# NIRVANALAN/GaussianAnything

Hardware: NVIDIA H100
Metric: 512^2 views/sec @100k Gaussians (surfel raster fwd+bwd) (higher is better)
Workload: dtype f32

## Files before the change

### gaussiananything_b200/csrc/raster_api.cu

```cuda
#include "../../include/ga_b200.h"
#include "raster_common.cuh"

static size_t align_up(size_t x, size_t a) { return (x + a - 1) / a * a; }

static int g_profile = 0;
static cudaEvent_t g_ev[7];
static bool g_ev_init = false;
static inline void prof(int i, cudaStream_t s) { if (g_profile) cudaEventRecord(g_ev[i], s); }

extern "C" int ga_profile_enable(int on)
{
    if (on && !g_ev_init) {
        for (int i = 0; i < 7; i++)
            if (cudaEventCreate(&g_ev[i]) != cudaSuccess) return GA_ERR_BADARG;
        g_ev_init = true;
    }
    g_profile = on ? 1 : 0;
    return 0;
}

extern "C" int ga_profile_read(float *ms, int n)
{
    if (!g_ev_init || !ms || n < 5) return 0;
    if (cudaEventSynchronize(g_ev[6]) != cudaSuccess) return 0;
// ... 33 lines not shown
}

extern "C" int ga_raster_layout_ex(int batch, int P, int views, int H, int W,
                                   int64_t max_instances, int list_k, GaRasterLayout *L)
{
    RasterDims d;
    int rc = make_dims(batch, P, views, H, W, 1.0f, max_instances, &d, list_k);
    if (rc) return rc;
    if (!L) return GA_ERR_BADARG;
    const size_t NVP = (size_t)d.NV * P, NVT = (size_t)d.NV * d.T, HW = (size_t)H * W;
    const size_t mi = (size_t)(max_instances > 0 ? max_instances : 1);
    size_t off = 0;
    L->status = off;     off = align_up(off + 16 * sizeof(int32_t), 256);
    L->rec = off;        off = align_up(off + NVP * GA_REC_F * sizeof(float), 256);
    L->depth = off;      off = align_up(off + NVP * sizeof(float), 256);
    L->rect = off;       off = align_up(off + NVP * sizeof(uint32_t), 256);
    L->tile_count = off; off = align_up(off + NVT * (GA_TILE_REPLICAS + 1) * sizeof(uint32_t), 256);
    L->tile_start = off; off = align_up(off + (NVT + 1) * sizeof(uint32_t), 256);
    L->keys = off;       off = align_up(off + mi * sizeof(uint64_t), 256);
    L->ids = off;        off = align_up(off + mi * sizeof(uint32_t), 256);
    L->final_T = off;    off = align_up(off + (size_t)d.NV * 3 * HW * sizeof(float), 256);
    L->n_contrib = off;  off = align_up(off + (size_t)d.NV * 2 * HW * sizeof(int32_t), 256);
    L->inst_cnt = off;   off = align_up(off + mi * sizeof(uint32_t), 256);
    L->n_list = off;     off = align_up(off + (list_k ? (size_t)d.NV * HW * sizeof(int32_t) : 0), 256);
    L->tile_flag = off;  off = align_up(off + (list_k ? NVT * sizeof(uint32_t) : 0), 256);
    L->lists = off;      off = align_up(off + (size_t)list_k * NVT * 256 * 16, 256);
    L->total_bytes = off;
    return 0;
}

static void carve(const GaRasterLayout &L, const RasterDims &d, void *base, RasterWs *w)
{
    char *p = (char *)base;
    w->status = (int32_t *)(p + L.status);
    w->rec = (float *)(p + L.rec);
    w->depth = (float *)(p + L.depth);
    w->rect = (uint32_t *)(p + L.rect);
    w->tile_count = (uint32_t *)(p + L.tile_count);
    w->big_tiles = w->tile_count + (size_t)d.NV * d.T * GA_TILE_REPLICAS;
    w->tile_start = (uint32_t *)(p + L.tile_start);
    w->keys = (unsigned long long *)(p + L.keys);
    w->ids = (uint32_t *)(p + L.ids);
    w->final_T = (float *)(p + L.final_T);
    w->n_contrib = (int32_t *)(p + L.n_contrib);
    w->inst_cnt = (uint32_t *)(p + L.inst_cnt);
    w->n_list = (int32_t *)(p + L.n_list);
    w->tile_flag = (uint32_t *)(p + L.tile_flag);
    w->lists = (uint4 *)(p + L.lists);
}

extern "C" int ga_raster_forward_ex(const float *gauss13, int batch, int P, int views,
                                    const float *viewmats, const float *projmats, const float *bg,
                                    int H, int W, float scale_modifier,
                                    float *out_color, float *out_allmap, int32_t *out_radii,
                                    void *workspace, size_t workspace_bytes, int64_t max_instances, int list_k,
                                    int32_t *status_host, void *status_event, void *stream)
{
    if ((status_host == nullptr) != (status_event == nullptr)) return GA_ERR_BADARG;
    RasterDims d;
    int rc = make_dims(batch, P, views, H, W, scale_modifier, max_instances, &d, list_k);
    if (rc) return rc;
    if (!gauss13 || !viewmats || !projmats || !bg || !out_color || !out_allmap || !out_radii || !workspace)
        return GA_ERR_BADARG;
    GaRasterLayout L;
    ga_raster_layout_ex(batch, P, views, H, W, max_instances, list_k, &L);
    if (workspace_bytes < L.total_bytes) return GA_ERR_WORKSPACE;
    RasterWs w;
    carve(L, d, workspace, &w);
    cudaStream_t s = (cudaStream_t)stream;
    cudaError_t e;
    if ((e = cudaMemsetAsync(w.status, 0, 16 * sizeof(int32_t), s)) != cudaSuccess) return (int)e;
    if ((e = cudaMemsetAsync(w.tile_count, 0, (size_t)d.NV * d.T * GA_TILE_REPLICAS * sizeof(uint32_t), s)) != cudaSuccess) return (int)e;
    prof(0, s);
    if ((e = ga_launch_preprocess(d, w, gauss13, viewmats, projmats, out_radii, s)) != cudaSuccess) return (int)e;
    prof(1, s);
    if ((e = ga_launch_binning(d, w, s, status_host, (cudaEvent_t)status_event)) != cudaSuccess) return (int)e;
    prof(2, s);
    if (list_k && (e = cudaMemsetAsync(w.tile_flag, 0, (size_t)d.NV * d.T * sizeof(uint32_t), s)) != cudaSuccess) return (int)e;
    if ((e = ga_launch_render_fwd(d, w, bg, out_color, out_allmap, s)) != cudaSuccess) return (int)e;
    prof(3, s);
    return 0;
}

static size_t bwd_acc_bytes(int batch, int P, int views) { return align_up((size_t)batch * views * P * GA_GRAD_F * sizeof(float), 256); }

extern "C" size_t ga_raster_backward_scratch_bytes(int batch, int P, int views)
{
    if (batch <= 0 || P <= 0 || views <= 0) return 0;
    return bwd_acc_bytes(batch, P, views);
}

extern "C" int ga_raster_backward_ex(const float *gauss13, int batch, int P, int views,
                                     const float *viewmats, const float *projmats, const float *bg,
                                     int H, int W, float scale_modifier,
                                     const int32_t *radii,
                                     const float *dL_dcolor, const float *dL_dallmap,
                                     const void *workspace, size_t workspace_bytes, int64_t max_instances, int list_k,
                                     void *scratch, size_t scratch_bytes,
                                     float *grad_gauss13, void *stream)
{
    RasterDims d;
    int rc = make_dims(batch, P, views, H, W, scale_modifier, max_instances, &d, list_k);
    if (rc) return rc;
    if (!gauss13 || !viewmats || !projmats || !bg || !radii || !dL_dcolor || !dL_dallmap ||
        !workspace || !scratch || !grad_gauss13)
        return GA_ERR_BADARG;
    GaRasterLayout L;
    ga_raster_layout_ex(batch, P, views, H, W, max_instances, list_k, &L);
    if (workspace_bytes < L.total_bytes) return GA_ERR_WORKSPACE;
    const size_t need = bwd_acc_bytes(batch, P, views);
    if (scratch_bytes < need) return GA_ERR_WORKSPACE;
    RasterWs w;
    carve(L, d, const_cast<void *>(workspace), &w);
    cudaStream_t s = (cudaStream_t)stream;
    cudaError_t e;
    float *grad_acc = (float *)scratch;
    prof(4, s);
    if ((e = cudaMemsetAsync(grad_acc, 0, need, s)) != cudaSuccess) return (int)e;
    if ((e = ga_launch_render_bwd(d, w, bg, dL_dcolor, dL_dallmap, grad_acc, s)) != cudaSuccess) return (int)e;
    prof(5, s);
    if ((e = ga_launch_preprocess_bwd(d, w, gauss13, viewmats, projmats, radii, grad_acc, grad_gauss13, s)) != cudaSuccess)
        return (int)e;
    prof(6, s);
    return 0;
}

extern "C" const char *ga_b200_version(void) { return "ga_b200 0.2 (sm_90a)"; }
```

### gaussiananything_b200/csrc/raster_common.cuh

```cuda
#pragma once
#include <cuda_runtime.h>
#include <stdint.h>

#define GA_BLOCK_X 16
#define GA_BLOCK_Y 16
#define GA_NEAR_N 0.2f
#define GA_FAR_N 100.0f
#define GA_FILTER_SIZE 0.707106f
#define GA_FILTER_INV_SQUARE 2.0f
#define GA_CUTOFF 3.0f
#define GA_REC_F 24
#define GA_GRAD_F 18


struct RasterDims {
    int batch, P, views, NV;
    int H, W, gx, gy, T;
    float scale_modifier;
    int64_t max_instances;
    int list_k;
    int radius_formula;
    int quat_norm_grad;
};
#ifndef GA_RADIUS_FORMULA
#define GA_RADIUS_FORMULA 0
#endif
#ifndef GA_QUAT_NORM_GRAD
#define GA_QUAT_NORM_GRAD 0
#endif

struct RasterWs {
    int32_t *status;
    float *rec;
    float *depth;
    uint32_t *rect;
    uint32_t *tile_count;
    uint32_t *big_tiles;
    uint32_t *tile_start;
    unsigned long long *keys;
    uint32_t *ids;
    float *final_T;
    int32_t *n_contrib;
    uint4 *lists;
    int32_t *n_list;
    uint32_t *tile_flag;
    uint32_t *inst_cnt;
};

cudaError_t ga_launch_preprocess(const RasterDims &d, const RasterWs &w, const float *gauss13,
                                 const float *viewmats, const float *projmats,
                                 int32_t *out_radii, cudaStream_t s);
#ifndef GA_TILE_REPLICAS
#define GA_TILE_REPLICAS 8
#endif

cudaError_t ga_launch_binning(const RasterDims &d, const RasterWs &w, cudaStream_t s, int32_t *status_host,
                              cudaEvent_t status_event);
cudaError_t ga_launch_render_fwd(const RasterDims &d, const RasterWs &w, const float *bg,
                                 float *out_color, float *out_allmap, cudaStream_t s);
cudaError_t ga_launch_render_bwd(const RasterDims &d, const RasterWs &w, const float *bg,
                                 const float *dL_dcolor, const float *dL_dallmap,
                                 float *grad_acc, cudaStream_t s);
cudaError_t ga_launch_preprocess_bwd(const RasterDims &d, const RasterWs &w, const float *gauss13,
                                     const float *viewmats, const float *projmats,
                                     const int32_t *radii, const float *grad_acc,
                                     float *grad_gauss13, cudaStream_t s);
```

### gaussiananything_b200/csrc/raster_preprocess.cu

```cuda
#include "raster_common.cuh"

__device__ __forceinline__ void quat_to_rotmat(const float *q, float R[3][3])
{
    float n2 = ((q[0] * q[0] + q[1] * q[1]) + q[2] * q[2]) + q[3] * q[3];
    float s = 1.0f / sqrtf(n2);
    float w = q[0] * s, x = q[1] * s, y = q[2] * s, z = q[3] * s;
    R[0][0] = 1.f - 2.f * (y * y + z * z);
    R[1][0] = 2.f * (x * y + w * z);
    R[2][0] = 2.f * (x * z - w * y);
    R[0][1] = 2.f * (x * y - w * z);
    R[1][1] = 1.f - 2.f * (x * x + z * z);
    R[2][1] = 2.f * (y * z + w * x);
    R[0][2] = 2.f * (x * z + w * y);
    R[1][2] = 2.f * (y * z - w * x);
    R[2][2] = 1.f - 2.f * (x * x + y * y);
}

__device__ __forceinline__ void surfel_transmat(const float R[3][3], float sx, float sy, float px, float py, float pz,
                                                const float *pm, int W, int H, float Tu[3], float Tv[3], float Tw[3])
{
    float L0[3] = {R[0][0] * sx, R[1][0] * sx, R[2][0] * sx};
    float L1[3] = {R[0][1] * sy, R[1][1] * sy, R[2][1] * sy};
    const float hw = 0.5f * (float)W, hh = 0.5f * (float)H;
    const float cw = 0.5f * (float)(W - 1), ch = 0.5f * (float)(H - 1);
// ... 96 lines not shown
                            float hx = sqrtf(fmaxf(0.f, qx)) * 1.01f + 0.51f;
                            float hy = sqrtf(fmaxf(0.f, qy)) * 1.01f + 0.51f;
                            bx0 = fminf(bx0, ccx - hx); bx1 = fmaxf(bx1, ccx + hx);
                            by0 = fminf(by0, ccy - hy); by1 = fmaxf(by1, ccy + hy);
                        } else {
                            bx0 = -1e30f; bx1 = 1e30f; by0 = -1e30f; by1 = 1e30f;
                        }
                    }
                    rec[16] = bx0; rec[17] = bx1; rec[18] = by0; rec[19] = by1;
                }
            }
        }
    }
    out_radii[vi] = radius_i;
    ws.depth[vi] = depth_out;
    ws.rect[vi] = rect_packed;
#pragma unroll
    for (int q = 0; q < GA_REC_F / 4; q++)
        rec_out[q] = make_float4(rec[4 * q], rec[4 * q + 1], rec[4 * q + 2], rec[4 * q + 3]);
    if (radius_i > 0) {
        const int x0 = rect_packed & 255, y0 = (rect_packed >> 8) & 255;
        const int x1 = (rect_packed >> 16) & 255, y1 = rect_packed >> 24;
        uint32_t *tc = ws.tile_count + (size_t)view * d.T * GA_TILE_REPLICAS + ((threadIdx.x >> 5) & (GA_TILE_REPLICAS - 1));
        for (int y = y0; y < y1; y++)
            for (int x = x0; x < x1; x++) atomicAdd(&tc[(y * d.gx + x) * GA_TILE_REPLICAS], 1u);
    }
}

__global__ void __launch_bounds__(256, 4)
preprocess_kernel(RasterDims d, RasterWs ws, const float *__restrict__ gauss13,
                  const float *__restrict__ viewmats, const float *__restrict__ projmats,
                  int32_t *__restrict__ out_radii)
{
    __shared__ float s_g[256 * 13];
    __shared__ float s_cam[32];
    __shared__ float4 s_rec[256 * GA_REC_F / 4];
    const int view = blockIdx.y;
    const int b = view / d.views;
    const int i0 = blockIdx.x * 256;
    const int n = min(256, d.P - i0);
    const float *src = gauss13 + ((size_t)b * d.P + i0) * 13;
    for (int t = threadIdx.x; t < n * 13; t += 256) s_g[t] = src[t];
    if (threadIdx.x < 16) s_cam[threadIdx.x] = viewmats[view * 16 + threadIdx.x];
    else if (threadIdx.x < 32) s_cam[threadIdx.x] = projmats[view * 16 + threadIdx.x - 16];
    __syncthreads();
    if ((int)threadIdx.x < n) preprocess_one(d, ws, s_g + threadIdx.x * 13, s_cam, view, i0 + threadIdx.x,
                                             s_rec + threadIdx.x * (GA_REC_F / 4), out_radii);
    __syncthreads();
    float4 *dst = reinterpret_cast<float4 *>(ws.rec + ((size_t)view * d.P + i0) * GA_REC_F);
    for (int t = threadIdx.x; t < n * (GA_REC_F / 4); t += 256) dst[t] = s_rec[t];
}

cudaError_t ga_launch_preprocess(const RasterDims &d, const RasterWs &w, const float *gauss13,
                                 const float *viewmats, const float *projmats,
                                 int32_t *out_radii, cudaStream_t s)
{
    dim3 grid((d.P + 255) / 256, d.NV);
    preprocess_kernel<<<grid, 256, 0, s>>>(d, w, gauss13, viewmats, projmats, out_radii);
    return cudaGetLastError();
}

__global__ void __launch_bounds__(256)
preprocess_bwd_kernel(RasterDims d, RasterWs ws, const float *__restrict__ gauss13,
                      const float *__restrict__ viewmats, const float *__restrict__ projmats,
                      const int32_t *__restrict__ radii, const float *__restrict__ grad_acc,
                      float *__restrict__ grad_gauss13)
{
    const int b = blockIdx.y;
    const int i = blockIdx.x * 256 + threadIdx.x;
    if (i >= d.P) return;
    const float *g = gauss13 + ((size_t)b * d.P + i) * 13;
    float q[4] = {g[6], g[7], g[8], g[9]};
    float R[3][3];
    quat_to_rotmat(q, R);
    const float sx = d.scale_modifier * g[4], sy = d.scale_modifier * g[5];
    const float px = g[0], py = g[1], pz = g[2];
    const float hw = 0.5f * d.W, hh = 0.5f * d.H, cw = 0.5f * (d.W - 1), ch = 0.5f * (d.H - 1);
    float gm[3] = {0, 0, 0}, gs[2] = {0, 0}, dR[3][3] = {{0, 0, 0}, {0, 0, 0}, {0, 0, 0}};
    float gop = 0.f, gcol[3] = {0, 0, 0};
    for (int v = 0; v < d.views; v++) {
        const int view = b * d.views + v;
        const size_t vi = (size_t)view * d.P + i;
        if (!(radii[vi] > 0)) continue;
        const float *ga = grad_acc + vi * GA_GRAD_F;
        const float *vm = viewmats + view * 16, *pm = projmats + view * 16;
        float G[3][3];
#pragma unroll
        for (int c = 0; c < 3; c++)
#pragma unroll
            for (int r = 0; r < 3; r++) G[c][r] = ga[3 * c + r];
        const float gmx = ga[9], gmy = ga[10];
        if (gmx != 0.f || gmy != 0.f) {
            const float t[3] = {9.f, 9.f, -1.f};
            float Tu[3], Tv[3], Tw[3];
            surfel_transmat(R, sx, sy, px, py, pz, pm, d.W, d.H, Tu, Tv, Tw);
            float dd = 0.f;
#pragma unroll
            for (int r = 0; r < 3; r++) dd += t[r] * Tw[r] * Tw[r];
            float f[3], dL_dd = 0.f;
#pragma unroll
            for (int r = 0; r < 3; r++) f[r] = t[r] / dd;
#pragma unroll
            for (int r = 0; r < 3; r++) {
                G[0][r] += gmx * f[r] * Tw[r];
                G[1][r] += gmy * f[r] * Tw[r];
                G[2][r] += gmx * f[r] * Tu[r] + gmy * f[r] * Tv[r];
                dL_dd += (gmx * Tu[r] * Tw[r] + gmy * Tv[r] * Tw[r]) * f[r];
            }
            dL_dd *= (-1.0f / dd);
#pragma unroll
            for (int r = 0; r < 3; r++) G[2][r] += dL_dd * t[r] * Tw[r] * 2.0f;
        }
        float dM[3][3];
#pragma unroll
        for (int k = 0; k < 3; k++) {
            float an0 = pm[4 * k + 0] * hw + pm[4 * k + 3] * cw;
            float an1 = pm[4 * k + 1] * hh + pm[4 * k + 3] * ch;
            float an2 = pm[4 * k + 3];
#pragma unroll
            for (int r = 0; r < 3; r++) dM[r][k] = an0 * G[0][r] + an1 * G[1][r] + an2 * G[2][r];
        }
        float vx = ((vm[0] * px + vm[4] * py) + vm[8] * pz) + vm[12];
        float vy = ((vm[1] * px + vm[5] * py) + vm[9] * pz) + vm[13];
        float vz = ((vm[2] * px + vm[6] * py) + vm[10] * pz) + vm[14];
        float nx = (vm[0] * R[0][2] + vm[4] * R[1][2]) + vm[8] * R[2][2];
        float ny = (vm[1] * R[0][2] + vm[5] * R[1][2]) + vm[9] * R[2][2];
        float nz = (vm[2] * R[0][2] + vm[6] * R[1][2]) + vm[10] * R[2][2];
        float cosv = -((vx * nx + vy * ny) + vz * nz);
        const float mult = cosv > 0.f ? 1.f : -1.f;
        const float gn0 = ga[11], gn1 = ga[12], gn2 = ga[13];
        float dtn[3];
        dtn[0] = mult * (vm[0] * gn0 + vm[1] * gn1 + vm[2] * gn2);
        dtn[1] = mult * (vm[4] * gn0 + vm[5] * gn1 + vm[6] * gn2);
        dtn[2] = mult * (vm[8] * gn0 + vm[9] * gn1 + vm[10] * gn2);
#pragma unroll
        for (int k = 0; k < 3; k++) {
            dR[k][0] += dM[0][k] * sx;
            dR[k][1] += dM[1][k] * sy;
            dR[k][2] += dtn[k];
            gs[0] += dM[0][k] * R[k][0];
            gs[1] += dM[1][k] * R[k][1];
            gm[k] += dM[2][k];
        }
        gop += ga[14];
        gcol[0] += ga[15]; gcol[1] += ga[16]; gcol[2] += ga[17];
    }
    float n2 = q[0] * q[0] + q[1] * q[1] + q[2] * q[2] + q[3] * q[3];
    float s = rsqrtf(n2);
    float w = q[0] * s, x = q[1] * s, y = q[2] * s, z = q[3] * s;
    float gw = 2 * (z * (dR[1][0] - dR[0][1]) + y * (dR[0][2] - dR[2][0]) + x * (dR[2][1] - dR[1][2]));
    float gxq = 2 * (-2 * x * (dR[1][1] + dR[2][2]) + y * (dR[1][0] + dR[0][1]) + z * (dR[2][0] + dR[0][2]) + w * (dR[2][1] - dR[1][2]));
    float gyq = 2 * (x * (dR[1][0] + dR[0][1]) - 2 * y * (dR[0][0] + dR[2][2]) + z * (dR[2][1] + dR[1][2]) + w * (dR[0][2] - dR[2][0]));
    float gzq = 2 * (x * (dR[2][0] + dR[0][2]) + y * (dR[2][1] + dR[1][2]) - 2 * z * (dR[0][0] + dR[1][1]) + w * (dR[1][0] - dR[0][1]));
    if (d.quat_norm_grad) {
        const float dot = w * gw + x * gxq + y * gyq + z * gzq;
        gw = (gw - w * dot) * s; gxq = (gxq - x * dot) * s; gyq = (gyq - y * dot) * s; gzq = (gzq - z * dot) * s;
    }
    float *o = grad_gauss13 + ((size_t)b * d.P + i) * 13;
    o[0] = gm[0]; o[1] = gm[1]; o[2] = gm[2];
    o[3] = gop;
    o[4] = d.scale_modifier * gs[0]; o[5] = d.scale_modifier * gs[1];
    o[6] = gw; o[7] = gxq; o[8] = gyq; o[9] = gzq;
    o[10] = gcol[0]; o[11] = gcol[1]; o[12] = gcol[2];
}

cudaError_t ga_launch_preprocess_bwd(const RasterDims &d, const RasterWs &w, const float *gauss13,
                                     const float *viewmats, const float *projmats,
// ... 9 lines not shown
```

### gaussiananything_b200/csrc/raster_render.cu

```cuda
#include "raster_common.cuh"
#include "device_once.cuh"

#define CHUNK 256

__device__ __forceinline__ float fast_rcp(float x)
{
    float r;
    asm("rcp.approx.ftz.f32 %0, %1;" : "=f"(r) : "f"(x));
    return r;
}
__device__ __forceinline__ float fast_ex2(float x)
{
    float r;
    asm("ex2.approx.ftz.f32 %0, %1;" : "=f"(r) : "f"(x));
    return r;
}
#define GA_M_C0 (GA_FAR_N / (GA_FAR_N - GA_NEAR_N))
#define GA_M_C1 (GA_FAR_N * GA_NEAR_N / (GA_FAR_N - GA_NEAR_N))
#define GA_NEG_HALF_LOG2E (-0.72134752044448170368f)

struct PixelGeom {
    float s0, s1, p2, rho3d, rho2d, dx, dy, depth, G, alpha;
    bool use3d;
};
// ... 98 lines not shown
            const TileBox q = clip_box(bb, ox, oy, min(ox + 15, d.W - 1), min(oy + 15, d.H - 1));
            npairs = q.w * q.h;
            sm.box[threadIdx.x] = npairs ? (uint32_t)(q.x0 | q.y0 << 4 | q.w << 8 | (65536 / q.w + 1) << 13) : 0u;
        }
        int incl = npairs;
#pragma unroll
        for (int o = 1; o < 32; o <<= 1) {
            const int y = __shfl_up_sync(0xffffffffu, incl, o);
            if (lane >= o) incl += y;
        }
        if (lane == 31) sm.wsum[warp] = incl;
        __syncthreads();
#pragma unroll
        for (int k = 0; k < 8; k++) incl += k < warp ? sm.wsum[k] : 0;
        sm.base[threadIdx.x] = incl - npairs;
        if (threadIdx.x == CHUNK - 1) sm.base[CHUNK] = incl;

        int t0 = 0, base = 0;
        while (t0 < cnt) {
#pragma unroll
            for (int k = 0; k < CHUNK / 32; k++) sm.mask[k][threadIdx.x] = 0u;
            const int t1 = t0 + __syncthreads_count((int)threadIdx.x >= t0 && (int)threadIdx.x < cnt &&
                                                    incl - base <= FWD_PAIRS);
            const int wpairs = sm.base[t1] - base;
            for (int q = threadIdx.x; q < wpairs; q += 256) {
                const int Q = base + q;
                int jj = t0;
#pragma unroll
                for (int step = CHUNK / 2; step > 0; step >>= 1)
                    if (jj + step < t1 && sm.base[jj + step] <= Q) jj += step;
                const uint32_t bx = sm.box[jj];
                const int k = Q - sm.base[jj], w = (bx >> 8) & 31;
                const int ry = (k * (int)(bx >> 13)) >> 16;
                const int lx = (int)(bx & 15) + k - ry * w, ly = (int)((bx >> 4) & 15) + ry;
                const float dxf = (float)lx, dyf = (float)ly;
                const float4 f0 = sm.rec[0][jj], f1 = sm.rec[1][jj], f2 = sm.rec[2][jj], f3 = sm.rec[3][jj];
                const float p0 = f0.x + dxf * f0.w + dyf * f1.z;
                const float p1 = f0.y + dxf * f1.x + dyf * f1.w;
                const float p2 = f0.z + dxf * f1.y + dyf * f2.x;
                const float ip = fast_rcp(p2);
                const float s0 = p0 * ip, s1 = p1 * ip;
                const float rho3d = s0 * s0 + s1 * s1;
                const float ddx = f3.x - dxf, ddy = f3.y - dyf;
                const float rho2d = GA_FILTER_INV_SQUARE * __fmaf_rn(ddx, ddx, __fmul_rn(ddy, ddy));
                const float rho = fminf(rho3d, rho2d);
                const float depth = (rho3d <= rho2d) ? (s0 * f2.y + s1 * f2.z) + f2.w : f2.w;
                const float alpha = fminf(0.99f, f3.z * fast_ex2(rho * GA_NEG_HALF_LOG2E));
                if (p2 != 0.0f && depth >= GA_NEAR_N && alpha >= 1.0f / 255.0f) {
                    sm.pair[q] = make_float2(alpha, depth);
                    atomicOr(&sm.mask[jj >> 5][ly * 16 + lx], 1u << (jj & 31));
                }
            }
            __syncthreads();
            if (!done) {
                int wi = t0 >> 5;
                const int wlast = (t1 - 1) >> 5;
                uint32_t m = sm.mask[wi][pix_local];
                while (true) {
                    while (m == 0u && wi < wlast) m = sm.mask[++wi][pix_local];
                    if (m == 0u) break;
                    const int jj = wi * 32 + __ffs(m) - 1;
                    m &= m - 1;
                    const uint32_t bx = sm.box[jj];
                    const int k = (lyi - (int)((bx >> 4) & 15)) * (int)((bx >> 8) & 31) + (lxi - (int)(bx & 15));
                    const float2 ad = sm.pair[sm.base[jj] - base + k];
                    const float alpha = ad.x, depth = ad.y;
                    const float test_T = T * (1 - alpha);
                    if (test_T < 0.0001f) { done = true; break; }
                    const float4 nr = sm.rec[4][jj], gb = sm.rec[5][jj];
                    const int contributor = c0 + jj + 1;
                    const float w = alpha * T;
                    const float A = 1 - T;
                    const float mm = GA_M_C0 - GA_M_C1 * fast_rcp(depth);
                    dist += (mm * mm * A + M2 - 2 * mm * M1) * w;
                    Dacc += depth * w;
                    M1 += mm * w;
                    M2 += mm * mm * w;
                    if (T > 0.5f) { median_depth = depth; median_contributor = contributor; }
                    N0 += nr.x * w; N1 += nr.y * w; N2 += nr.z * w;
                    C0 += nr.w * w; C1 += gb.x * w; C2 += gb.y * w;
                    T = test_T;
                    last_contributor = contributor;
                    if (LISTS) {
                        atomicAdd(&sm.cnt[jj], 1);
                        if (nl < d.list_k)
                            my_list[(size_t)nl * 256] = make_uint4((uint32_t)(contributor - 1), __float_as_uint(alpha),
                                                                   __float_as_uint(depth), 0u);
                        nl++;
                    }
                }
            }
            t0 = t1;
            if (t0 < cnt) base = sm.base[t0];
            if (__syncthreads_count(done) == 256) break;
        }
        if (LISTS && (int)threadIdx.x < cnt) ws.inst_cnt[start + c0 + threadIdx.x] = (uint32_t)sm.cnt[threadIdx.x];
    }
    if (LISTS) {
        if (inside) ws.n_list[(size_t)view * d.H * d.W + (size_t)pyi * d.W + pxi] = nl;
        if (nl > d.list_k) ws.tile_flag[(size_t)view * d.T + tile] = 1u;
    }
    if (inside) {
        const size_t HW = (size_t)d.H * d.W;
        const size_t pix = (size_t)pyi * d.W + pxi;
        float *fT = ws.final_T + (size_t)view * 3 * HW;
        int32_t *nc = ws.n_contrib + (size_t)view * 2 * HW;
        fT[pix] = T; fT[pix + HW] = M1; fT[pix + 2 * HW] = M2;
        nc[pix] = last_contributor; nc[pix + HW] = median_contributor;
        float *oc = out_color + (size_t)view * 3 * HW;
        oc[pix] = C0 + T * bg[0]; oc[pix + HW] = C1 + T * bg[1]; oc[pix + 2 * HW] = C2 + T * bg[2];
        float *oa = out_allmap + (size_t)view * 7 * HW;
        oa[pix] = Dacc;
        oa[pix + HW] = 1 - T;
        oa[pix + 2 * HW] = N0; oa[pix + 3 * HW] = N1; oa[pix + 4 * HW] = N2;
        oa[pix + 5 * HW] = median_depth;
        oa[pix + 6 * HW] = dist;
    }
}

cudaError_t ga_launch_render_fwd(const RasterDims &d, const RasterWs &w, const float *bg,
                                 float *out_color, float *out_allmap, cudaStream_t s)
{
    static GaPerDevice attr_set;
    if (ga_first_use_on_device(attr_set)) {
        cudaError_t e = cudaFuncSetAttribute(render_fwd_kernel<true>, cudaFuncAttributeMaxDynamicSharedMemorySize,
                                             (int)sizeof(FwdSmem));
        if (e == cudaSuccess)
            e = cudaFuncSetAttribute(render_fwd_kernel<false>, cudaFuncAttributeMaxDynamicSharedMemorySize,
                                     (int)sizeof(FwdSmem));
        if (e != cudaSuccess) return e;
    }
    dim3 grid(d.gx, d.gy, d.NV);
    if (d.list_k > 0) render_fwd_kernel<true><<<grid, 256, sizeof(FwdSmem), s>>>(d, w, bg, out_color, out_allmap);
    else render_fwd_kernel<false><<<grid, 256, sizeof(FwdSmem), s>>>(d, w, bg, out_color, out_allmap);
    return cudaGetLastError();
}

#define BWD_RECORDS 4096
#define BWD_TPI 2

struct BwdSmem {
    float4 rec[6][CHUNK];
    uint4 recs[BWD_RECORDS];
    float4 up[3][256];
    uint32_t id[CHUNK];
    int off[CHUNK];
    int cnt[CHUNK];
    int bin[64];
    uint16_t perm[CHUNK];
    int wsum[8];
    int maxc, m;
};

template <int TPI>
__device__ __forceinline__ void reduce_scatter18(const float (&g)[GA_GRAD_F], int lane, float *__restrict__ dst)
{
    int off = 0, size = 9;
    float a9[10];
    {
        const bool u = lane & (TPI >> 1);
#pragma unroll
        for (int i = 0; i < 9; i++) {
            const float keep = u ? g[9 + i] : g[i], send = u ? g[i] : g[9 + i];
            a9[i] = keep + __shfl_xor_sync(0xffffffffu, send, TPI >> 1);
        }
        a9[9] = 0.f;
        off += u ? 9 : 0;
    }
    if constexpr (TPI == 2) {
#pragma unroll
        for (int i = 0; i < 9; i++)
            if (a9[i] != 0.f) atomicAdd(dst + off + i, a9[i]);
        return;
    } else {
        float b5[6];
        {
            const bool u = lane & (TPI >> 2);
#pragma unroll
            for (int i = 0; i < 5; i++) {
                const float keep = u ? a9[5 + i] : a9[i], send = u ? a9[i] : a9[5 + i];
                b5[i] = keep + __shfl_xor_sync(0xffffffffu, send, TPI >> 2);
            }
            b5[5] = 0.f;
            off += u ? 5 : 0; size = u ? 4 : 5;
        }
        if constexpr (TPI == 4) {
#pragma unroll
            for (int i = 0; i < 5; i++)
                if (i < size && b5[i] != 0.f) atomicAdd(dst + off + i, b5[i]);
            return;
        } else {
            float c3[4];
            {
                const bool u = lane & (TPI >> 3);
#pragma unroll
                for (int i = 0; i < 3; i++) {
                    const float keep = u ? b5[3 + i] : b5[i], send = u ? b5[i] : b5[3 + i];
                    c3[i] = keep + __shfl_xor_sync(0xffffffffu, send, TPI >> 3);
                }
                c3[3] = 0.f;
                off += u ? 3 : 0; size = u ? size - 3 : 3;
            }
            if constexpr (TPI == 8) {
#pragma unroll
                for (int i = 0; i < 3; i++)
                    if (i < size && c3[i] != 0.f) atomicAdd(dst + off + i, c3[i]);
                return;
            } else {
                const bool u = lane & (TPI >> 4);
                float d2[2];
#pragma unroll
                for (int i = 0; i < 2; i++) {
                    const float keep = u ? c3[2 + i] : c3[i], send = u ? c3[i] : c3[2 + i];
                    d2[i] = keep + __shfl_xor_sync(0xffffffffu, send, TPI >> 4);
                }
                off += u ? 2 : 0; size = u ? max(size - 2, 0) : min(size, 2);
#pragma unroll
                for (int i = 0; i < 2; i++)
                    if (i < size && d2[i] != 0.f) atomicAdd(dst + off + i, d2[i]);
            }
        }
    }
}

__device__ __forceinline__ int clipped_box_area(const float4 bb, int ox, int oy)
{
    const TileBox q = clip_box(bb, ox, oy, ox + 15, oy + 15);
    return q.w * q.h;
}

template <bool LISTS>
__device__ __forceinline__ void bwd_tile(const RasterDims &d, const RasterWs &ws, BwdSmem &sm, const float *__restrict__ bg,
                                         const float *__restrict__ dL_dcolor, const float *__restrict__ dL_dallmap,
                                         float *__restrict__ grad_acc)
{
    const int view = blockIdx.z;
    const int tile = blockIdx.y * d.gx + blockIdx.x;
    const int warp = threadIdx.x >> 5, lane = threadIdx.x & 31;
    const int ox = blockIdx.x * GA_BLOCK_X, oy = blockIdx.y * GA_BLOCK_Y;
    const int lx0 = (warp & 1) * 8, ly0 = (warp >> 1) * 4;
    const int lxi = lx0 + (lane & 7), lyi = ly0 + (lane >> 3);
    const int pxi = ox + lxi, pyi = oy + lyi;
    const int pix_local = lyi * 16 + lxi;
    const bool inside = pxi < d.W && pyi < d.H;
    const float pfx = (float)pxi, pfy = (float)pyi;

    const uint32_t start = ws.tile_start[(size_t)view * d.T + tile];
    const size_t HW = (size_t)d.H * d.W;
    const size_t pix = inside ? (size_t)pyi * d.W + pxi : 0;
    const float *fT = ws.final_T + (size_t)view * 3 * HW;
    const int32_t *nc = ws.n_contrib + (size_t)view * 2 * HW;
    const float *rec_base = ws.rec + (size_t)view * d.P * GA_REC_F;
    float *acc_base = grad_acc + (size_t)view * d.P * GA_GRAD_F;

    const float T_final = inside ? fT[pix] : 0.f;
    float T = T_final;
    const int last_contributor = inside ? nc[pix] : 0;
    const int median_contributor = inside ? nc[pix + HW] : 0;
    float bg_dot_dpixel = 0.f;
    {
        float4 u0 = make_float4(0.f, 0.f, 0.f, 0.f), u1 = u0, u2 = u0;
        if (inside) {
            const float *gc = dL_dcolor + (size_t)view * 3 * HW;
            const float *ga = dL_dallmap + (size_t)view * 7 * HW;
            u0 = make_float4(gc[pix], gc[pix + HW], gc[pix + 2 * HW], ga[pix + 2 * HW]);
            u1 = make_float4(ga[pix + 3 * HW], ga[pix + 4 * HW], ga[pix], ga[pix + HW]);
            u2 = make_float4(ga[pix + 6 * HW], ga[pix + 5 * HW], fT[pix + HW], fT[pix + 2 * HW]);
        }
        sm.up[0][pix_local] = u0;
        sm.up[1][pix_local] = u1;
        sm.up[2][pix_local] = u2;
        bg_dot_dpixel = bg[0] * u0.x + bg[1] * u0.y + bg[2] * u0.z;
    }
    const float final_A = 1 - T_final;
    float last_alpha = 0, v_last = 0, v_acc = 0, last_dL_dT = 0;

    const uint4 *my_list = nullptr;
    int kk = -1;
    if (LISTS) {
        my_list = ws.lists + ((size_t)view * d.T + tile) * (size_t)d.list_k * 256 + pix_local;
        kk = (inside ? ws.n_list[(size_t)view * HW + pix] : 0) - 1;
#pragma unroll
        for (int q = 0; q < 8; q++)
            if (kk >= q) asm volatile("prefetch.global.L2 [%0];" ::"l"(my_list + (size_t)(kk - q) * 256));
    }

    if (threadIdx.x == 0) sm.maxc = 0;
    __syncthreads();
    {
        int mc = last_contributor;
#pragma unroll
        for (int o = 16; o > 0; o >>= 1) mc = max(mc, __shfl_xor_sync(0xffffffffu, mc, o));
        if (lane == 0) atomicMax(&sm.maxc, mc);
    }
    __syncthreads();
    const int total = sm.maxc;

    for (int hi = total; hi > 0; hi -= CHUNK) {
        const int cnt = min(CHUNK, hi);
        int bound = 0;
        if ((int)threadIdx.x < cnt) {
            const int pos = hi - 1 - (int)threadIdx.x;
            const uint32_t id = ws.ids[start + pos];
            sm.id[threadIdx.x] = id;
            const float4 *src = reinterpret_cast<const float4 *>(rec_base + (size_t)id * GA_REC_F);
            float4 q[6];
#pragma unroll
            for (int k = 0; k < 6; k++) { q[k] = __ldg(src + k); sm.rec[k][threadIdx.x] = q[k]; }
            bound = LISTS ? (int)ws.inst_cnt[start + pos] : clipped_box_area(q[4], ox, oy);
        }
        int incl = bound;
#pragma unroll
        for (int o = 1; o < 32; o <<= 1) {
            const int y = __shfl_up_sync(0xffffffffu, incl, o);
            if (lane >= o) incl += y;
        }
        if (lane == 31) sm.wsum[warp] = incl;
        __syncthreads();
#pragma unroll
        for (int k = 0; k < 8; k++) incl += k < warp ? sm.wsum[k] : 0;
        sm.off[threadIdx.x] = incl - bound;
        sm.cnt[threadIdx.x] = 0;

        int t0 = 0, base = 0;
        while (t0 < cnt) {
            if (threadIdx.x < 64) sm.bin[threadIdx.x] = 0;
            const int t1 = t0 + __syncthreads_count((int)threadIdx.x >= t0 && (int)threadIdx.x < cnt &&
                                                    incl - base <= BWD_RECORDS);

            auto contribute = [&](const int jj, const int contributor, const float alpha, const float c_d) {
                const float4 nr = sm.rec[3][jj], gb = sm.rec[5][jj];
                const float4 u0 = sm.up[0][pix_local], u1 = sm.up[1][pix_local], u2 = sm.up[2][pix_local];
                const float dL_ddepth = u1.z, dL_dreg = u2.x, final_D = u2.z, final_D2 = u2.w;
                const float inv1ma = fast_rcp(1.f - alpha);
                T = T * inv1ma;
                const float w = alpha * T;
                float dL_dz = 0.0f;
                const float inv_cd = fast_rcp(c_d);
                const float m_d = GA_M_C0 - GA_M_C1 * inv_cd;
                const float dmd_dd = GA_M_C1 * inv_cd * inv_cd;
                if (contributor == median_contributor - 1) dL_dz += u2.y;
                const float dL_dweight = (final_D2 + m_d * m_d * final_A - 2 * m_d * final_D) * dL_dreg;
                const float dL_dmd = 2.0f * (T * alpha) * (m_d * final_A - final_D) * dL_dreg;
                dL_dz += dL_dmd * dmd_dd;
                const float v = ((nr.w * u0.x + gb.x * u0.y) + (gb.y * u0.z + c_d * dL_ddepth)) +
                                ((nr.x * u0.w + nr.y * u1.x) + (nr.z * u1.y + u1.w));
                v_acc = last_alpha * v_last + (1.f - last_alpha) * v_acc;
                v_last = v;
                float dL_dalpha = (v - v_acc) + (dL_dweight - last_dL_dT);
                last_dL_dT = dL_dweight * alpha + (1 - alpha) * last_dL_dT;
                dL_dalpha *= T;
                last_alpha = alpha;
                dL_dalpha += (-T_final * inv1ma) * bg_dot_dpixel;
                dL_dz += w * dL_ddepth;
                const int slot = atomicAdd(&sm.cnt[jj], 1);
                sm.recs[sm.off[jj] - base + slot] =
                    make_uint4((uint32_t)pix_local, __float_as_uint(dL_dalpha), __float_as_uint(dL_dz), __float_as_uint(w));
            };
            if constexpr (LISTS) {
                const int pos_lo = hi - t1;
                uint4 e = make_uint4(0u, 0u, 0u, 0u), e1 = e, e2 = e;
                if (kk >= 0) e = __ldg(my_list + (size_t)kk * 256);
                if (kk >= 1) e1 = __ldg(my_list + (size_t)(kk - 1) * 256);
                if (kk >= 2) e2 = __ldg(my_list + (size_t)(kk - 2) * 256);
                while (true) {
                    const bool active = kk >= 0 && (int)e.x >= pos_lo;
                    if (!__any_sync(0xffffffffu, active)) break;
                    if (active) {
                        const uint4 cur = e;
                        e = e1; e1 = e2;
                        if (kk >= 3) e2 = __ldg(my_list + (size_t)(kk - 3) * 256);
                        if (kk >= 8) asm volatile("prefetch.global.L2 [%0];" ::"l"(my_list + (size_t)(kk - 8) * 256));
                        kk--;
                        contribute(hi - 1 - (int)cur.x, (int)cur.x, __uint_as_float(cur.y), __uint_as_float(cur.z));
                    }
                }
            } else {
                const float bx_lo = (float)(ox + lx0), bx_hi = (float)(ox + lx0 + 7);
                const float by_lo = (float)(oy + ly0), by_hi = (float)(oy + ly0 + 3);
                for (int sb = t0; sb < t1; sb += 32) {
                    bool hit = false;
                    if (sb + lane < t1) {
                        const float4 bb = sm.rec[4][sb + lane];
                        hit = !(bb.y < bx_lo || bb.x > bx_hi || bb.w < by_lo || bb.z > by_hi);
                    }
                    unsigned mask = __ballot_sync(0xffffffffu, hit);
                    unsigned mine = 0;
                    while (mask) {
                        const int b = __ffs(mask) - 1;
                        mask &= mask - 1;
                        const float4 bb = sm.rec[4][sb + b];
                        if (pfx >= bb.x && pfx <= bb.y && pfy >= bb.z && pfy <= bb.w && (hi - 1 - (sb + b)) < last_contributor)
                            mine |= 1u << b;
                    }
                    if (!inside) mine = 0;
                    while (__any_sync(0xffffffffu, mine != 0)) {
                        const bool active = mine != 0;
                        const int bsel = active ? __ffs(mine) - 1 : 0;
                        mine &= mine - 1;
                        const int jj = sb + bsel;
                        const float4 a = sm.rec[0][jj], b = sm.rec[1][jj], c = sm.rec[2][jj];
                        PixelGeom pg;
                        float k0, k1, k2, l0, l1, l2;
                        const bool ok = active && eval_pair(a, b, c, pfx, pfy, pg, k0, k1, k2, l0, l1, l2);
                        if (ok) contribute(jj, hi - 1 - jj, pg.alpha, pg.depth);
                    }
                }
            }
            __syncthreads();

            const int myc = ((int)threadIdx.x >= t0 && (int)threadIdx.x < t1) ? sm.cnt[threadIdx.x] : 0;
            if (myc > 0) atomicAdd(&sm.bin[min(myc, 63)], 1);
            __syncthreads();
            if (threadIdx.x < 32) {
                const int hi_bin = 63 - 2 * (int)threadIdx.x, lo_bin = hi_bin - 1;
                const int vh = sm.bin[hi_bin], vl = lo_bin >= 1 ? sm.bin[lo_bin] : 0;
                int x = vh + vl;
#pragma unroll
                for (int o = 1; o < 32; o <<= 1) {
                    const int y = __shfl_up_sync(0xffffffffu, x, o);
                    if ((int)threadIdx.x >= o) x += y;
                }
                const int excl = x - (vh + vl);
                sm.bin[hi_bin] = excl;
                if (lo_bin >= 1) sm.bin[lo_bin] = excl + vh;
                if (threadIdx.x == 31) sm.m = x;
            }
            __syncthreads();
            if (myc > 0) sm.perm[atomicAdd(&sm.bin[min(myc, 63)], 1)] = (uint16_t)threadIdx.x;
            __syncthreads();
            const int m = sm.m, sub = threadIdx.x % BWD_TPI;
            for (int b0 = 0; b0 < m; b0 += 256 / BWD_TPI) {
                const int slot = b0 + (int)threadIdx.x / BWD_TPI;
                const int jj = slot < m ? (int)sm.perm[slot] : 0;
                const int n = slot < m ? sm.cnt[jj] : 0;
                float g[GA_GRAD_F];
#pragma unroll
                for (int f = 0; f < GA_GRAD_F; f++) g[f] = 0.f;
                if (n > 0) {
                    const float4 a = sm.rec[0][jj], b = sm.rec[1][jj], c = sm.rec[2][jj];
                    const float opa = c.w;
                    const uint4 *lst = sm.recs + (sm.off[jj] - base);
                    for (int r = sub; r < n; r += BWD_TPI) {
                        const uint4 rc = lst[r];
                        const int p = (int)rc.x;
                        const float dL_dalpha = __uint_as_float(rc.y), dL_dz = __uint_as_float(rc.z), w = __uint_as_float(rc.w);
                        const float qx = (float)(ox + (p & 15)), qy = (float)(oy + (p >> 4));
                        PixelGeom pg;
                        float k0, k1, k2, l0, l1, l2;
                        eval_pair(a, b, c, qx, qy, pg, k0, k1, k2, l0, l1, l2);
                        const float G = pg.G;
                        const float dL_dG = opa * dL_dalpha;
                        if (pg.use3d) {
                            const float dL_ds0 = dL_dG * -G * pg.s0 + dL_dz * b.z;
                            const float dL_ds1 = dL_dG * -G * pg.s1 + dL_dz * b.w;
                            const float ip = fast_rcp(pg.p2);
                            const float q0 = dL_ds0 * ip, q1 = dL_ds1 * ip;
                            const float q2 = -(q0 * pg.s0 + q1 * pg.s1);
                            const float dk0 = l1 * q2 - l2 * q1, dk1 = l2 * q0 - l0 * q2, dk2 = l0 * q1 - l1 * q0;
                            const float dl0 = q1 * k2 - q2 * k1, dl1 = q2 * k0 - q0 * k2, dl2 = q0 * k1 - q1 * k0;
                            g[0] -= dk0; g[1] -= dk1; g[2] -= dk2;
                            g[3] -= dl0; g[4] -= dl1; g[5] -= dl2;
                            g[6] += qx * dk0 + qy * dl0 + dL_dz * pg.s0;
                            g[7] += qx * dk1 + qy * dl1 + dL_dz * pg.s1;
                            g[8] += qx * dk2 + qy * dl2 + dL_dz;
                        } else {
                            g[9] += dL_dG * (-G * GA_FILTER_INV_SQUARE * pg.dx);
                            g[10] += dL_dG * (-G * GA_FILTER_INV_SQUARE * pg.dy);
                            g[8] += dL_dz;
                        }
                        g[14] += G * dL_dalpha;
                        const float4 ua = sm.up[0][p], ub = sm.up[1][p];
                        g[15] += w * ua.x; g[16] += w * ua.y; g[17] += w * ua.z;
                        g[11] += w * ua.w; g[12] += w * ub.x; g[13] += w * ub.y;
                    }
                }
                if (__any_sync(0xffffffffu, n > 0))
                    reduce_scatter18<BWD_TPI>(g, lane, acc_base + (size_t)(n > 0 ? sm.id[jj] : 0) * GA_GRAD_F);
            }
            t0 = t1;
            if (t0 < cnt) base = sm.off[t0];
            __syncthreads();
        }
    }
}

__global__ void __launch_bounds__(256, 2)
render_bwd_kernel(RasterDims d, RasterWs ws, const float *__restrict__ bg, const float *__restrict__ dL_dcolor,
                  const float *__restrict__ dL_dallmap, float *__restrict__ grad_acc)
{
    extern __shared__ __align__(16) uint8_t bwd_smem_raw[];
    BwdSmem &sm = *reinterpret_cast<BwdSmem *>(bwd_smem_raw);
    if (ws.status[1]) return;
    if (d.list_k > 0 && ws.tile_flag[(size_t)blockIdx.z * d.T + blockIdx.y * d.gx + blockIdx.x] == 0)
        bwd_tile<true>(d, ws, sm, bg, dL_dcolor, dL_dallmap, grad_acc);
    else
        bwd_tile<false>(d, ws, sm, bg, dL_dcolor, dL_dallmap, grad_acc);
}

cudaError_t ga_launch_render_bwd(const RasterDims &d, const RasterWs &w, const float *bg,
                                 const float *dL_dcolor, const float *dL_dallmap, float *grad_acc, cudaStream_t s)
{
    static GaPerDevice attr_set;
    if (ga_first_use_on_device(attr_set)) {
        cudaError_t e = cudaFuncSetAttribute(render_bwd_kernel, cudaFuncAttributeMaxDynamicSharedMemorySize,
                                             (int)sizeof(BwdSmem));
        if (e != cudaSuccess) return e;
    }
    dim3 grid(d.gx, d.gy, d.NV);
    render_bwd_kernel<<<grid, 256, sizeof(BwdSmem), s>>>(d, w, bg, dL_dcolor, dL_dallmap, grad_acc);
    return cudaGetLastError();
}
```

Before: 6325.

## Pad gradient rows to 20 floats and use vector reductions in backward

Pads each per-Gaussian gradient accumulator row from 18 to 20 floats so the backward render can flush pair-reduced gradients with 128-bit red.global.add.v4.f32 instead of many scalar atomics, and preprocess backward reads rows as float4. In the list path, the forward pass now stores each contributor's rank in the list record and the backward counts are precomputed from the list bounds. This lets the slot sort run before contribution and removes the per-record shared atomic on the count. It costs extra accumulator memory plus a hard BWD_TPI==2 assumption, and depends on v4 float reduction support (sm_90+).

```diff
diff --git a/gaussiananything_b200/csrc/raster_api.cu b/gaussiananything_b200/csrc/raster_api.cu
--- a/gaussiananything_b200/csrc/raster_api.cu
+++ b/gaussiananything_b200/csrc/raster_api.cu
@@ -139,7 +139,7 @@
     return 0;
 }
 
-static size_t bwd_acc_bytes(int batch, int P, int views) { return align_up((size_t)batch * views * P * GA_GRAD_F * sizeof(float), 256); }
+static size_t bwd_acc_bytes(int batch, int P, int views) { return align_up((size_t)batch * views * P * GA_GRAD_STRIDE * sizeof(float), 256); }
 
 extern "C" size_t ga_raster_backward_scratch_bytes(int batch, int P, int views)
 {
diff --git a/gaussiananything_b200/csrc/raster_common.cuh b/gaussiananything_b200/csrc/raster_common.cuh
--- a/gaussiananything_b200/csrc/raster_common.cuh
+++ b/gaussiananything_b200/csrc/raster_common.cuh
@@ -11,6 +11,7 @@
 #define GA_CUTOFF 3.0f
 #define GA_REC_F 24
 #define GA_GRAD_F 18
+#define GA_GRAD_STRIDE 20
 
 
 struct RasterDims {
diff --git a/gaussiananything_b200/csrc/raster_preprocess.cu b/gaussiananything_b200/csrc/raster_preprocess.cu
--- a/gaussiananything_b200/csrc/raster_preprocess.cu
+++ b/gaussiananything_b200/csrc/raster_preprocess.cu
@@ -202,7 +202,10 @@
         const int view = b * d.views + v;
         const size_t vi = (size_t)view * d.P + i;
         if (!(radii[vi] > 0)) continue;
-        const float *ga = grad_acc + vi * GA_GRAD_F;
+        alignas(16) float ga[GA_GRAD_STRIDE];
+        const float4 *row = reinterpret_cast<const float4 *>(grad_acc + vi * GA_GRAD_STRIDE);
+#pragma unroll
+        for (int k = 0; k < GA_GRAD_STRIDE / 4; k++) reinterpret_cast<float4 *>(ga)[k] = __ldg(row + k);
         const float *vm = viewmats + view * 16, *pm = projmats + view * 16;
         float G[3][3];
 #pragma unroll
diff --git a/gaussiananything_b200/csrc/raster_render.cu b/gaussiananything_b200/csrc/raster_render.cu
--- a/gaussiananything_b200/csrc/raster_render.cu
+++ b/gaussiananything_b200/csrc/raster_render.cu
@@ -204,10 +204,10 @@
                     T = test_T;
                     last_contributor = contributor;
                     if (LISTS) {
-                        atomicAdd(&sm.cnt[jj], 1);
+                        const int rank = atomicAdd(&sm.cnt[jj], 1);
                         if (nl < d.list_k)
                             my_list[(size_t)nl * 256] = make_uint4((uint32_t)(contributor - 1), __float_as_uint(alpha),
-                                                                   __float_as_uint(depth), 0u);
+                                                                   __float_as_uint(depth), (uint32_t)rank);
                         nl++;
                     }
                 }
@@ -274,75 +274,28 @@
     int maxc, m;
 };
 
-template <int TPI>
-__device__ __forceinline__ void reduce_scatter18(const float (&g)[GA_GRAD_F], int lane, float *__restrict__ dst)
-{
-    int off = 0, size = 9;
-    float a9[10];
-    {
-        const bool u = lane & (TPI >> 1);
-#pragma unroll
-        for (int i = 0; i < 9; i++) {
-            const float keep = u ? g[9 + i] : g[i], send = u ? g[i] : g[9 + i];
-            a9[i] = keep + __shfl_xor_sync(0xffffffffu, send, TPI >> 1);
-        }
-        a9[9] = 0.f;
-        off += u ? 9 : 0;
-    }
-    if constexpr (TPI == 2) {
-#pragma unroll
-        for (int i = 0; i < 9; i++)
-            if (a9[i] != 0.f) atomicAdd(dst + off + i, a9[i]);
-        return;
-    } else {
-        float b5[6];
-        {
-            const bool u = lane & (TPI >> 2);
-#pragma unroll
-            for (int i = 0; i < 5; i++) {
-                const float keep = u ? a9[5 + i] : a9[i], send = u ? a9[i] : a9[5 + i];
-                b5[i] = keep + __shfl_xor_sync(0xffffffffu, send, TPI >> 2);
-            }
-            b5[5] = 0.f;
-            off += u ? 5 : 0; size = u ? 4 : 5;
-        }
-        if constexpr (TPI == 4) {
-#pragma unroll
-            for (int i = 0; i < 5; i++)
-                if (i < size && b5[i] != 0.f) atomicAdd(dst + off + i, b5[i]);
-            return;
-        } else {
-            float c3[4];
-            {
-                const bool u = lane & (TPI >> 3);
-#pragma unroll
-                for (int i = 0; i < 3; i++) {
-                    const float keep = u ? b5[3 + i] : b5[i], send = u ? b5[i] : b5[3 + i];
-                    c3[i] = keep + __shfl_xor_sync(0xffffffffu, send, TPI >> 3);
-                }
-                c3[3] = 0.f;
-                off += u ? 3 : 0; size = u ? size - 3 : 3;
-            }
-            if constexpr (TPI == 8) {
-#pragma unroll
-                for (int i = 0; i < 3; i++)
-                    if (i < size && c3[i] != 0.f) atomicAdd(dst + off + i, c3[i]);
-                return;
-            } else {
-                const bool u = lane & (TPI >> 4);
-                float d2[2];
-#pragma unroll
-                for (int i = 0; i < 2; i++) {
-                    const float keep = u ? c3[2 + i] : c3[i], send = u ? c3[i] : c3[2 + i];
-                    d2[i] = keep + __shfl_xor_sync(0xffffffffu, send, TPI >> 4);
-                }
-                off += u ? 2 : 0; size = u ? max(size - 2, 0) : min(size, 2);
-#pragma unroll
-                for (int i = 0; i < 2; i++)
-                    if (i < size && d2[i] != 0.f) atomicAdd(dst + off + i, d2[i]);
-            }
-        }
-    }
+__device__ __forceinline__ void red_add_v4(float *dst, const float4 v)
+{
+    asm volatile("red.relaxed.gpu.global.add.v4.f32 [%0], {%1, %2, %3, %4};"
+                 ::"l"(dst), "f"(v.x), "f"(v.y), "f"(v.z), "f"(v.w) : "memory");
+}
+
+static_assert(BWD_TPI == 2, "phase B reduces over lane pairs");
+__device__ __forceinline__ void reduce_pair_add(const float (&g)[GA_GRAD_F], int lane, float *__restrict__ dst)
+{
+    const bool odd = lane & 1;
+    float k[10];
+#pragma unroll
+    for (int i = 0; i < 10; i++) {
+        const float ge = g[i < 8 ? i : 8 + i];
+        const float go = i < 8 ? g[8 + i] : 0.f;
+        k[i] = (odd ? go : ge) + __shfl_xor_sync(0xffffffffu, odd ? ge : go, 1);
+    }
+    const float4 v0 = make_float4(k[0], k[1], k[2], k[3]), v1 = make_float4(k[4], k[5], k[6], k[7]);
+    float *row = dst + (odd ? 8 : 0);
+    if (v0.x != 0.f || v0.y != 0.f || v0.z != 0.f || v0.w != 0.f) red_add_v4(row, v0);
+    if (v1.x != 0.f || v1.y != 0.f || v1.z != 0.f || v1.w != 0.f) red_add_v4(row + 4, v1);
+    if (!odd && (k[8] != 0.f || k[9] != 0.f)) red_add_v4(dst + 16, make_float4(k[8], k[9], 0.f, 0.f));
 }
 
 __device__ __forceinline__ int clipped_box_area(const float4 bb, int ox, int oy)
@@ -373,7 +326,7 @@
     const float *fT = ws.final_T + (size_t)view * 3 * HW;
     const int32_t *nc = ws.n_contrib + (size_t)view * 2 * HW;
     const float *rec_base = ws.rec + (size_t)view * d.P * GA_REC_F;
-    float *acc_base = grad_acc + (size_t)view * d.P * GA_GRAD_F;
+    float *acc_base = grad_acc + (size_t)view * d.P * GA_GRAD_STRIDE;
 
     const float T_final = inside ? fT[pix] : 0.f;
     float T = T_final;
@@ -442,15 +395,38 @@
 #pragma unroll
         for (int k = 0; k < 8; k++) incl += k < warp ? sm.wsum[k] : 0;
         sm.off[threadIdx.x] = incl - bound;
-        sm.cnt[threadIdx.x] = 0;
+        sm.cnt[threadIdx.x] = LISTS ? bound : 0;
 
         int t0 = 0, base = 0;
         while (t0 < cnt) {
             if (threadIdx.x < 64) sm.bin[threadIdx.x] = 0;
             const int t1 = t0 + __syncthreads_count((int)threadIdx.x >= t0 && (int)threadIdx.x < cnt &&
                                                     incl - base <= BWD_RECORDS);
-
-            auto contribute = [&](const int jj, const int contributor, const float alpha, const float c_d) {
+            const bool in_window = (int)threadIdx.x >= t0 && (int)threadIdx.x < t1;
+
+            auto sort_slots = [&](const int myc) {
+                if (myc > 0) atomicAdd(&sm.bin[min(myc, 63)], 1);
+                __syncthreads();
+                if (threadIdx.x < 32) {
+                    const int hi_bin = 63 - 2 * (int)threadIdx.x, lo_bin = hi_bin - 1;
+                    const int vh = sm.bin[hi_bin], vl = lo_bin >= 1 ? sm.bin[lo_bin] : 0;
+                    int x = vh + vl;
+#pragma unroll
+                    for (int o = 1; o < 32; o <<= 1) {
+                        const int y = __shfl_up_sync(0xffffffffu, x, o);
+                        if ((int)threadIdx.x >= o) x += y;
+                    }
+                    const int excl = x - (vh + vl);
+                    sm.bin[hi_bin] = excl;
+                    if (lo_bin >= 1) sm.bin[lo_bin] = excl + vh;
+                    if (threadIdx.x == 31) sm.m = x;
+                }
+                __syncthreads();
+                if (myc > 0) sm.perm[atomicAdd(&sm.bin[min(myc, 63)], 1)] = (uint16_t)threadIdx.x;
+            };
+            if constexpr (LISTS) sort_slots(in_window ? bound : 0);
+
+            auto contribute = [&](const int jj, const int contributor, const float alpha, const float c_d, const int rank) {
                 const float4 nr = sm.rec[3][jj], gb = sm.rec[5][jj];
                 const float4 u0 = sm.up[0][pix_local], u1 = sm.up[1][pix_local], u2 = sm.up[2][pix_local];
                 const float dL_ddepth = u1.z, dL_dreg = u2.x, final_D = u2.z, final_D2 = u2.w;
@@ -475,7 +451,8 @@
                 last_alpha = alpha;
                 dL_dalpha += (-T_final * inv1ma) * bg_dot_dpixel;
                 dL_dz += w * dL_ddepth;
-                const int slot = atomicAdd(&sm.cnt[jj], 1);
+                int slot = rank;
+                if constexpr (!LISTS) slot = atomicAdd(&sm.cnt[jj], 1);
                 sm.recs[sm.off[jj] - base + slot] =
                     make_uint4((uint32_t)pix_local, __float_as_uint(dL_dalpha), __float_as_uint(dL_dz), __float_as_uint(w));
             };
@@ -494,7 +471,7 @@
                         if (kk >= 3) e2 = __ldg(my_list + (size_t)(kk - 3) * 256);
                         if (kk >= 8) asm volatile("prefetch.global.L2 [%0];" ::"l"(my_list + (size_t)(kk - 8) * 256));
                         kk--;
-                        contribute(hi - 1 - (int)cur.x, (int)cur.x, __uint_as_float(cur.y), __uint_as_float(cur.z));
+                        contribute(hi - 1 - (int)cur.x, (int)cur.x, __uint_as_float(cur.y), __uint_as_float(cur.z), (int)cur.w);
                     }
                 }
             } else {
@@ -525,32 +502,17 @@
                         PixelGeom pg;
                         float k0, k1, k2, l0, l1, l2;
                         const bool ok = active && eval_pair(a, b, c, pfx, pfy, pg, k0, k1, k2, l0, l1, l2);
-                        if (ok) contribute(jj, hi - 1 - jj, pg.alpha, pg.depth);
+                        if (ok) contribute(jj, hi - 1 - jj, pg.alpha, pg.depth, 0);
                     }
                 }
             }
             __syncthreads();
 
-            const int myc = ((int)threadIdx.x >= t0 && (int)threadIdx.x < t1) ? sm.cnt[threadIdx.x] : 0;
-            if (myc > 0) atomicAdd(&sm.bin[min(myc, 63)], 1);
-            __syncthreads();
-            if (threadIdx.x < 32) {
-                const int hi_bin = 63 - 2 * (int)threadIdx.x, lo_bin = hi_bin - 1;
-                const int vh = sm.bin[hi_bin], vl = lo_bin >= 1 ? sm.bin[lo_bin] : 0;
-                int x = vh + vl;
-#pragma unroll
-                for (int o = 1; o < 32; o <<= 1) {
-                    const int y = __shfl_up_sync(0xffffffffu, x, o);
-                    if ((int)threadIdx.x >= o) x += y;
-                }
-                const int excl = x - (vh + vl);
-                sm.bin[hi_bin] = excl;
-                if (lo_bin >= 1) sm.bin[lo_bin] = excl + vh;
-                if (threadIdx.x == 31) sm.m = x;
+            if constexpr (!LISTS) {
+                sort_slots(in_window ? sm.cnt[threadIdx.x] : 0);
+                __syncthreads();
             }
-            __syncthreads();
-            if (myc > 0) sm.perm[atomicAdd(&sm.bin[min(myc, 63)], 1)] = (uint16_t)threadIdx.x;
-            __syncthreads();
+
             const int m = sm.m, sub = threadIdx.x % BWD_TPI;
             for (int b0 = 0; b0 < m; b0 += 256 / BWD_TPI) {
                 const int slot = b0 + (int)threadIdx.x / BWD_TPI;
@@ -598,7 +560,7 @@
                     }
                 }
                 if (__any_sync(0xffffffffu, n > 0))
-                    reduce_scatter18<BWD_TPI>(g, lane, acc_base + (size_t)(n > 0 ? sm.id[jj] : 0) * GA_GRAD_F);
+                    reduce_pair_add(g, lane, acc_base + (size_t)(n > 0 ? sm.id[jj] : 0) * GA_GRAD_STRIDE);
             }
             t0 = t1;
             if (t0 < cnt) base = sm.off[t0];
```

New measurement: 6441, median of 6. +1.8%, better.
